# nicholasburden/pymarl

Hardware: NVIDIA B200
Metric: qmix_learner_episodes_per_sec (higher is better)
Workload: dtype bf16 (fp32 accumulate)

## Files before the change

pymarl_b200/csrc/tc_common.cuh:

```cuda
#pragma once
#include <cuda_bf16.h>
#include <stdint.h>

namespace pmb {
namespace tc {

__device__ __forceinline__ uint32_t smem_u32(const void* p) { return (uint32_t)__cvta_generic_to_shared(p); }

__device__ __forceinline__ void mbar_init(uint64_t* bar, uint32_t count) {
    asm volatile("mbarrier.init.shared::cta.b64 [%0], %1;" ::"r"(smem_u32(bar)), "r"(count) : "memory");
}
__device__ __forceinline__ void fence_barrier_init() {
    asm volatile("fence.mbarrier_init.release.cluster;" ::: "memory");
}
__device__ __forceinline__ void mbar_arrive(uint64_t* bar) {
    asm volatile("mbarrier.arrive.shared::cta.b64 _, [%0];" ::"r"(smem_u32(bar)) : "memory");
}
__device__ __forceinline__ void mbar_arrive_expect_tx(uint64_t* bar, uint32_t bytes) {
    asm volatile("mbarrier.arrive.expect_tx.shared::cta.b64 _, [%0], %1;" ::"r"(smem_u32(bar)), "r"(bytes) : "memory");
}
__device__ __forceinline__ bool mbar_try_wait(uint64_t* bar, uint32_t parity) {
    uint32_t ok;
    asm volatile(
        "{\n\t.reg .pred p;\n\t"
// ... 61 lines not shown
__device__ __forceinline__ void tmem_dealloc(uint32_t taddr, uint32_t ncols) {
    asm volatile("tcgen05.dealloc.cta_group::1.sync.aligned.b32 %0, %1;" ::"r"(taddr), "r"(ncols) : "memory");
}
__device__ __forceinline__ void pdl_launch_dependents() { asm volatile("griddepcontrol.launch_dependents;" ::: "memory"); }
__device__ __forceinline__ void pdl_wait() { asm volatile("griddepcontrol.wait;" ::: "memory"); }

__device__ __forceinline__ void tc_fence_before() { asm volatile("tcgen05.fence::before_thread_sync;" ::: "memory"); }
__device__ __forceinline__ void tc_fence_after() { asm volatile("tcgen05.fence::after_thread_sync;" ::: "memory"); }
__device__ __forceinline__ void tmem_wait_ld() { asm volatile("tcgen05.wait::ld.sync.aligned;" ::: "memory"); }

__device__ __forceinline__ void tmem_ld_32x32(uint32_t taddr, uint32_t (&v)[32]) {
    asm volatile(
        "tcgen05.ld.sync.aligned.32x32b.x32.b32 "
        "{%0, %1, %2, %3, %4, %5, %6, %7, %8, %9, %10, %11, %12, %13, %14, %15, "
        "%16, %17, %18, %19, %20, %21, %22, %23, %24, %25, %26, %27, %28, %29, %30, %31}, [%32];"
        : "=r"(v[0]), "=r"(v[1]), "=r"(v[2]), "=r"(v[3]), "=r"(v[4]), "=r"(v[5]), "=r"(v[6]), "=r"(v[7]), "=r"(v[8]),
          "=r"(v[9]), "=r"(v[10]), "=r"(v[11]), "=r"(v[12]), "=r"(v[13]), "=r"(v[14]), "=r"(v[15]), "=r"(v[16]),
          "=r"(v[17]), "=r"(v[18]), "=r"(v[19]), "=r"(v[20]), "=r"(v[21]), "=r"(v[22]), "=r"(v[23]), "=r"(v[24]),
          "=r"(v[25]), "=r"(v[26]), "=r"(v[27]), "=r"(v[28]), "=r"(v[29]), "=r"(v[30]), "=r"(v[31])
        : "r"(taddr)
        : "memory");
}

__device__ __forceinline__ uint64_t umma_desc_sw128(uint32_t smem_addr, uint32_t lbo_bytes, uint32_t sbo_bytes) {
    return (uint64_t)((smem_addr >> 4) & 0x3FFF) | ((uint64_t)((lbo_bytes >> 4) & 0x3FFF) << 16) |
           ((uint64_t)((sbo_bytes >> 4) & 0x3FFF) << 32) | (1ull << 46) | (2ull << 61);
}
__host__ __device__ constexpr uint32_t umma_idesc_bf16(int M, int N, int a_mn_major, int b_mn_major) {
    return (1u << 4) | (1u << 7) | (1u << 10) | ((uint32_t)a_mn_major << 15) | ((uint32_t)b_mn_major << 16) |
           ((uint32_t)(N >> 3) << 17) | ((uint32_t)(M >> 4) << 24);
}

__device__ __forceinline__ void umma_bf16(uint32_t tmem_d, uint64_t a_desc, uint64_t b_desc, uint32_t idesc,
                                          uint32_t accumulate) {
    asm volatile(
        "{\n\t.reg .pred p;\n\t"
        "setp.ne.b32 p, %4, 0;\n\t"
        "tcgen05.mma.cta_group::1.kind::f16 [%0], %1, %2, %3, p;\n\t}"
        :
        : "r"(tmem_d), "l"(a_desc), "l"(b_desc), "r"(idesc), "r"(accumulate)
        : "memory");
}
__device__ __forceinline__ void umma_commit(uint64_t* bar) {
    asm volatile("tcgen05.commit.cta_group::1.mbarrier::arrive::one.shared::cluster.b64 [%0];" ::"r"(smem_u32(bar))
                 : "memory");
}

__device__ __forceinline__ uint32_t pack_bf16x2(float lo, float hi) {
    uint32_t r;
    asm("cvt.rn.bf16x2.f32 %0, %1, %2;" : "=r"(r) : "f"(hi), "f"(lo));
    return r;
}

__host__ __device__ __forceinline__ uint32_t sw128_offset(uint32_t r, uint32_t j) {
    return r * 128u + ((j ^ (r & 7u)) << 4);
}

}
}
```

pymarl_b200/csrc/tc_gemm.cu:

```cuda
#include <cstdlib>
#include <algorithm>
#include "common.cuh"
#include "tc_common.cuh"
#include "mixer_tc.cuh"

namespace pmb {
namespace tc {

constexpr int BM = 128;
constexpr int BK = 64;
constexpr int BN_MAX = 256;
constexpr int STAGES = 4;
constexpr int A_STAGE_BYTES = BM * 128;
constexpr int W_STAGE_BYTES = BN_MAX * 128;
constexpr int N_EPI_WARPS = 4, MMA_WARP = 4, WLOAD_WARP = 5, FIRST_PROD_WARP = 6, N_PROD_WARPS = 8;
constexpr int THREADS = 32 * (FIRST_PROD_WARP + N_PROD_WARPS);
constexpr int SMEM_BYTES = 1024  + STAGES * (A_STAGE_BYTES + W_STAGE_BYTES) + 256;

struct GemmParams {
    const float* A;
    RowMap amap;
    int64_t M;
    int K;
    int n_chunks;
// ... 438 lines not shown
constexpr int RPW = GROUP_ROWS / N_CONV;
constexpr int threads_for(int ns) { return 32 * (PROD_W + ns + N_CONV); }
static_assert(RPW >= 1 && RPW * N_CONV == GROUP_ROWS, "group rows must divide over the converter warps");
}

struct Fc1StreamParams {
    const int64_t* ep_index;
    const float* obs; int64_t obs_sb;
    const __nv_bfloat16* Wp;
    uint8_t* obs_img;
    int64_t R;
    int T, N, O, n_tiles, n_chunks, slot_bytes;
    int fold_id;
    const uint4* tab_act16;
    const float* tab_id;
    const int64_t* actions; int64_t actions_sb;
    const int64_t* filled;  int64_t filled_sb;
    uint8_t* x_on; uint8_t* x_tg;
    uint32_t* relu_mask;
    int use_act;
    int l2_prefetch;
    int n_nets;
    int t0;
};

__device__ __forceinline__ float lds_f32(uint32_t addr) {
    float v;
    asm volatile("ld.shared.f32 %0, [%1];" : "=f"(v) : "r"(addr));
    return v;
}
__device__ __forceinline__ void sts_b32(uint32_t addr, uint32_t v) {
    asm volatile("st.shared.b32 [%0], %1;" ::"r"(addr), "r"(v) : "memory");
}

#ifdef PMB_FC1_PROFILE
__device__ unsigned long long g_fc1_prof[16];
#define TWAIT(idx, bar, par) do { long long _t0 = clock64(); mbar_wait(bar, par); if (lane == 0) prof_acc[idx] += clock64() - _t0; } while (0)
#define TMARK(var) const long long var = clock64()
#define TADD(idx, expr) do { if (lane == 0) prof_acc[idx] += (expr); } while (0)
#else
#define TWAIT(idx, bar, par) mbar_wait(bar, par)
#define TMARK(var)
#define TADD(idx, expr)
#endif
template <int NC, int NS>
__global__ void __launch_bounds__(fs::threads_for(NS), 1) fc1_stream_kernel(Fc1StreamParams P) {
#ifdef PMB_FC1_PROFILE
    long long prof_acc[12] = {0, 0, 0, 0, 0, 0, 0, 0, 0, 0, 0, 0};
    const long long prof_t0 = clock64();
#endif
    using namespace fs;
    extern __shared__ uint8_t smem_raw[];
    uint8_t* smem = reinterpret_cast<uint8_t*>((reinterpret_cast<uintptr_t>(smem_raw) + 1023) & ~(uintptr_t)1023);
    constexpr int N_SLOTS = NS, N_PROD = NS, FIRST_CONV_W = PROD_W + NS;
    constexpr int tile_bytes = NC * A_STAGE_BYTES;
    const int w_chunk = P.n_nets == 2 ? A_STAGE_BYTES : A_STAGE_BYTES / 2;
    uint8_t* w_s = smem;
    uint8_t* a_s = smem + NC * w_chunk;
    uint8_t* stage = a_s + tile_bytes;
    int* rowoff = reinterpret_cast<int*>(stage + N_SLOTS * P.slot_bytes);
    int* rown = rowoff + N_SLOTS * GROUP_ROWS;
    uint64_t* bars = reinterpret_cast<uint64_t*>(rown + N_SLOTS * GROUP_ROWS);
    uint64_t* w_full = bars;
    uint64_t* st_full = bars + 1;
    uint64_t* st_empty = st_full + N_SLOTS;
    uint64_t* a_full = st_empty + N_SLOTS;
    uint64_t* a_free = a_full + 1;
    uint64_t* tfull = a_free + 1;
    uint64_t* tempty = tfull + 2;
    uint32_t* tmem_slot = reinterpret_cast<uint32_t*>(tempty + 2);

    const int warp = threadIdx.x >> 5, lane = threadIdx.x & 31;
    if (threadIdx.x == 0) {
        mbar_init(w_full, 1);
        for (int i = 0; i < N_SLOTS; ++i) { mbar_init(&st_full[i], 1); mbar_init(&st_empty[i], N_CONV); }
        mbar_init(a_full, N_CONV); mbar_init(a_free, 1);
        for (int i = 0; i < 2; ++i) { mbar_init(&tfull[i], 1); mbar_init(&tempty[i], N_EPI); }
        fence_barrier_init();
    }
    if (warp == MMA_W) tmem_alloc(tmem_slot, 256);
    tc_fence_before();
    __syncthreads();
    tc_fence_after();
    const uint32_t tmem_base = *tmem_slot;
    const int64_t n_items = (int64_t)P.T * P.n_tiles;
    pdl_launch_dependents();

    if (warp >= PROD_W && warp < PROD_W + N_PROD) {
        const int pw = warp - PROD_W;
        if (pw == 0 && lane == 0) {
            mbar_arrive_expect_tx(w_full, (uint32_t)(NC * w_chunk));
            for (int c = 0; c < NC; ++c)
                bulk_copy_g2s(w_s + c * w_chunk, reinterpret_cast<const uint8_t*>(P.Wp) + c * A_STAGE_BYTES, (uint32_t)w_chunk, w_full);
        }
        uint32_t git = 0;
        for (int64_t item = blockIdx.x; item < n_items; item += gridDim.x) {
            const int64_t t = item / P.n_tiles, tile = item - t * P.n_tiles;
            for (int g = 0; g < GROUPS; ++g, ++git) {
                const int slot = git % N_SLOTS;
                if (slot != pw) continue;
                TMARK(pp0);
                uint8_t* sl = stage + slot * P.slot_bytes;
                int* ro = rowoff + slot * GROUP_ROWS;
                int* rn = rown + slot * GROUP_ROWS;
                const int64_t p0 = tile * BM + g * GROUP_ROWS;
                int rows_here = P.R - p0 < GROUP_ROWS ? (int)(P.R - p0) : GROUP_ROWS;
                if (rows_here < 0) rows_here = 0;
                const uint32_t b0 = (uint32_t)p0 / (uint32_t)P.N;
                const int n00 = (int)((uint32_t)p0 - b0 * (uint32_t)P.N);
                int first_cnt = P.N - n00;
                if (first_cnt > rows_here) first_cnt = rows_here;
                const int lr = lane == 0 ? 0 : first_cnt + (lane - 1) * P.N;
                int cnt = lane == 0 ? first_cnt : (rows_here - lr < P.N ? rows_here - lr : P.N);
                if (cnt < 0) cnt = 0;
                const int n0 = lane == 0 ? n00 : 0;
                const char* ga = nullptr;
                uint32_t cur = 0, phase = 0, cp_bytes = 0;
                if (cnt > 0) {
                    ga = reinterpret_cast<const char*>(P.obs + ep_row(P.ep_index, (int64_t)b0 + lane) * P.obs_sb +
                                                       ((t + P.t0) * P.N + n0) * (int64_t)P.O);
                    phase = (uint32_t)(reinterpret_cast<uintptr_t>(ga) & 15);
                    cur = (((uint32_t)lr * P.O * 4u + 127u) & ~127u) + 320u * lane + (uint32_t)(reinterpret_cast<uintptr_t>(ga) & 127);
                    cp_bytes = (phase + (uint32_t)cnt * P.O * 4u + 15u) & ~15u;
                }
                const uint32_t tx = __reduce_add_sync(0xffffffffu, cp_bytes);
                if (P.l2_prefetch && cnt > 0 && item + (int64_t)P.l2_prefetch * gridDim.x < n_items) {
                    const int64_t item2 = item + (int64_t)P.l2_prefetch * gridDim.x;
                    const int64_t t2 = item2 / P.n_tiles, tile2 = item2 - t2 * P.n_tiles;
                    const int64_t q0 = tile2 * BM + g * GROUP_ROWS;
                    int rows2 = P.R - q0 < GROUP_ROWS ? (int)(P.R - q0) : GROUP_ROWS;
                    if (rows2 < 0) rows2 = 0;
                    const uint32_t c0 = (uint32_t)q0 / (uint32_t)P.N;
                    const int m00 = (int)((uint32_t)q0 - c0 * (uint32_t)P.N);
                    int fc = P.N - m00;
                    if (fc > rows2) fc = rows2;
                    const int lr2 = lane == 0 ? 0 : fc + (lane - 1) * P.N;
                    int cnt2 = lane == 0 ? fc : (rows2 - lr2 < P.N ? rows2 - lr2 : P.N);
                    if (cnt2 > 0) {
                        const char* gb = reinterpret_cast<const char*>(P.obs + ep_row(P.ep_index, (int64_t)c0 + lane) * P.obs_sb +
                                                                       ((t2 + P.t0) * P.N + (lane == 0 ? m00 : 0)) * (int64_t)P.O);
                        const uintptr_t a0 = (reinterpret_cast<uintptr_t>(gb) + 15) & ~(uintptr_t)15;
                        const uintptr_t a1 = (reinterpret_cast<uintptr_t>(gb) + (uint64_t)cnt2 * P.O * 4) & ~(uintptr_t)15;
                        if (a1 > a0)
                            asm volatile("cp.async.bulk.prefetch.L2.global [%0], %1;" ::"l"(a0), "r"((uint32_t)(a1 - a0)) : "memory");
                    }
                }
                const int rj = lane < first_cnt ? 0 : 1 + (lane - first_cnt) / P.N;
                const int lrj = rj == 0 ? 0 : first_cnt + (rj - 1) * P.N;
                const uint32_t cur_j = __shfl_sync(0xffffffffu, cur, rj & 31);
                TADD(10, clock64() - pp0);
                TWAIT(0, &st_empty[slot], ((git / N_SLOTS) & 1) ^ 1);
                TMARK(pp1);
                if (lane < GROUP_ROWS) {
                    ro[lane] = lane < rows_here ? (int)(cur_j + (uint32_t)(lane - lrj) * P.O * 4u) : -1;
                    rn[lane] = (rj == 0 ? n00 : 0) + (lane - lrj);
                }
                if (cnt > 0) bulk_copy_g2s(sl + cur - phase, ga - phase, cp_bytes, &st_full[slot]);
                __syncwarp();
                if (lane == 0) {
                    if (tx) mbar_arrive_expect_tx(&st_full[slot], tx); else mbar_arrive(&st_full[slot]);
                }
                TADD(11, clock64() - pp1);
            }
        }
    } else if (warp >= FIRST_CONV_W) {
        const int cw = warp - FIRST_CONV_W;
        constexpr int c_last = NC - 1;
        const bool okl0 = c_last * BK + 2 * lane < P.O, okl1 = c_last * BK + 2 * lane + 1 < P.O;
        const int j_pad = c_last * BK + 2 * lane - P.O;
        const uint32_t a_s_u32 = smem_u32(a_s);
        const uint32_t a_base = a_s_u32 + ((uint32_t)(lane >> 2) << 4) + (lane & 3) * 4;
        uint32_t git = 0, ti = 0;
        for (int64_t item = blockIdx.x; item < n_items; item += gridDim.x, ++ti) {
            for (int g = 0; g < GROUPS; ++g, ++git) {
                const int slot = git % N_SLOTS;
                TWAIT(1, &st_full[slot], (git / N_SLOTS) & 1);
                TMARK(pt1);
                const uint32_t sl = smem_u32(stage + slot * P.slot_bytes) + 8u * lane;
                int offs[RPW], nns[RPW];
#pragma unroll
                for (int rr = 0; rr < RPW; ++rr) {
                    offs[rr] = rowoff[slot * GROUP_ROWS + RPW * cw + rr];
                    nns[rr] = rown[slot * GROUP_ROWS + RPW * cw + rr];
                }
                float v0[RPW][NC], v1[RPW][NC];
                {
#pragma unroll
                    for (int rr = 0; rr < RPW; ++rr) {
                        const int off = offs[rr];
                        const bool real = off >= 0;
                        const uint32_t src = sl + (uint32_t)(real ? off : 0);
#pragma unroll
                        for (int c = 0; c < NC; ++c) {
                            v0[rr][c] = 0.f; v1[rr][c] = 0.f;
                            if (real && (c < c_last || okl0)) v0[rr][c] = lds_f32(src + c * 256);
                            if (real && (c < c_last || okl1)) v1[rr][c] = lds_f32(src + c * 256 + 4);
                        }
                    }
                    uint32_t pk[RPW][NC];
#pragma unroll
                    for (int rr = 0; rr < RPW; ++rr) {
                        const int off = offs[rr];
                        const int nn = nns[rr];
                        const bool fold = P.fold_id && off >= 0;
                        const bool hit0 = fold && j_pad >= 0 && (j_pad == nn || j_pad == P.N);
                        const bool hit1 = fold && j_pad + 1 >= 0 && (j_pad + 1 == nn || j_pad + 1 == P.N);
#pragma unroll
                        for (int c = 0; c < NC; ++c) {
                            float a = v0[rr][c], b = v1[rr][c];
                            if (c == c_last) { a = hit0 ? 1.0f : a; b = hit1 ? 1.0f : b; }
                            pk[rr][c] = pack_bf16x2(a, b);
                        }
                    }
                    __syncwarp();
                    if (lane == 0) mbar_arrive(&st_empty[slot]);
                    TMARK(pt2);
                    TADD(6, pt2 - pt1);
                    if (g == 0) TWAIT(2, a_free, (ti & 1) ^ 1);
#pragma unroll
                    for (int rr = 0; rr < RPW; ++rr) {
                        const uint32_t rt = (uint32_t)(g * GROUP_ROWS + RPW * cw + rr);
                        const uint32_t dst = (a_base + rt * 128u) ^ ((rt & 7u) << 4);
#pragma unroll
                        for (int c = 0; c < NC; ++c) sts_b32(dst + c * A_STAGE_BYTES, pk[rr][c]);
                        if (P.obs_img) {
                            uint8_t* img = P.obs_img + item * tile_bytes + (dst - a_s_u32);
#pragma unroll
                            for (int c = 0; c < NC; ++c) __stcs(reinterpret_cast<uint32_t*>(img + c * A_STAGE_BYTES), pk[rr][c]);
                        }
                    }
                    TADD(7, clock64() - pt2);
                }
            }
            fence_proxy_async_smem();
            __syncwarp();
            if (lane == 0) mbar_arrive(a_full);
        }
    } else if (warp == MMA_W) {
        if (lane == 0) {
            const uint32_t idesc = umma_idesc_bf16(BM, 64 * P.n_nets, 0, 0);
            mbar_wait(w_full, 0);
            uint32_t ti = 0;
            for (int64_t item = blockIdx.x; item < n_items; item += gridDim.x, ++ti) {
                const int b = ti & 1;
                TWAIT(3, a_full, ti & 1);
                TWAIT(4, &tempty[b], ((ti >> 1) & 1) ^ 1);
                tc_fence_after();
                const uint32_t tm = tmem_base + 128u * b;
#pragma unroll
                for (int c = 0; c < NC; ++c) {
                    const uint32_t a_addr = smem_u32(a_s + c * A_STAGE_BYTES), w_addr = smem_u32(w_s + c * w_chunk);
#pragma unroll
                    for (int kk = 0; kk < BK / 16; ++kk)
                        umma_bf16(tm, umma_desc_sw128(a_addr + kk * 32, 16, 1024), umma_desc_sw128(w_addr + kk * 32, 16, 1024),
                                  idesc, (c | kk) != 0);
                }
                umma_commit(a_free);
                umma_commit(&tfull[b]);
            }
        }
// ... 51 lines not shown
                        if (tid) {
                            const float4 b0 = __ldg(tid + 2 * q), b1 = __ldg(tid + 2 * q + 1);
                            o[0] += b0.x; o[1] += b0.y; o[2] += b0.z; o[3] += b0.w;
                            o[4] += b1.x; o[5] += b1.y; o[6] += b1.z; o[7] += b1.w;
                        }
#pragma unroll
                        for (int k = 0; k < 8; ++k) {
                            o[k] = fmaxf(o[k], 0.f);
                            mbits |= (o[k] > 0.f ? 1u : 0u) << (8 * q + k);
                        }
                        *reinterpret_cast<uint4*>(tile_img + sw128_offset(r, (uint32_t)(h0 / 8 + q))) =
                            make_uint4(pack_bf16x2(o[0], o[1]), pack_bf16x2(o[2], o[3]), pack_bf16x2(o[4], o[5]),
                                       pack_bf16x2(o[6], o[7]));
                    }
                    if (P.relu_mask && net == 0) P.relu_mask[(item * 2 + (h0 >> 5)) * 128 + r] = mbits;
                }
            }
            tc_fence_before();
            __syncwarp();
            if (lane == 0) mbar_arrive(&tempty[b]);
            a_prev = a_next; n_cur = n_nxt;
        }
    }
#ifdef PMB_FC1_PROFILE
    if (lane == 0) {
        for (int i = 0; i < 8; ++i) if (prof_acc[i]) atomicAdd(&g_fc1_prof[i], (unsigned long long)prof_acc[i]);
        for (int i = 10; i < 12; ++i) if (prof_acc[i]) atomicAdd(&g_fc1_prof[i], (unsigned long long)prof_acc[i]);
        if (threadIdx.x == 0) { atomicAdd(&g_fc1_prof[8], (unsigned long long)(clock64() - prof_t0)); atomicAdd(&g_fc1_prof[9], 1ull); }
    }
#endif
    tc_fence_before();
    __syncthreads();
    if (warp == MMA_W) {
        tc_fence_after();
        tmem_dealloc(tmem_base, 256);
    }
}

}

int64_t tc_packed_elems(int Ncols, int K) {
    int n_chunks = (K + tc::BK - 1) / tc::BK;
    return (int64_t)Ncols * n_chunks * tc::BK;
}

int tc_pack_w(const float* const* ptrs, const int* rows, const int* lds, int nseg, int K, __nv_bfloat16* out,
              cudaStream_t s, int n_chunks_min) {
    tc::PackSegs segs;
    int Ncols = 0;
    segs.nseg = nseg;
    for (int i = 0; i < 4; ++i) {
        segs.ptr[i] = i < nseg ? ptrs[i] : nullptr;
        segs.rows[i] = i < nseg ? rows[i] : 0;
        segs.ld[i] = i < nseg ? lds[i] : 0;
        Ncols += segs.rows[i];
    }
    Ncols = (int)align_up(Ncols, 32);
    int n_chunks = (K + tc::BK - 1) / tc::BK;
// ... 126 lines not shown
                         reinterpret_cast<uint8_t*>(x_on), reinterpret_cast<uint8_t*>(x_tg), t0, nt, d->N, d->A,
                         d->obs_last_action, n_tiles, R, relu_mask};
        const int n_chunks = (d->O + tc::BK - 1) / tc::BK;
        const int slot_bytes = slot_bytes_s;
        const int64_t smem_need = 1024 + 2 * (int64_t)n_chunks * tc::A_STAGE_BYTES + tc::fs::N_SLOTS * (int64_t)slot_bytes +
                                  2 * tc::fs::N_SLOTS * tc::fs::GROUP_ROWS * 4 + 256;
        if (n_chunks <= tc::fs::MAX_CHUNKS && smem_need <= 232448) {
            const int fold_id = n_chunks * tc::BK - d->O >= d->N + 1;
            __nv_bfloat16* tab_act16 = reinterpret_cast<__nv_bfloat16*>(static_cast<char*>(scratch) + wp_bytes + ta_bytes + ti_bytes);
            const int64_t n_pack = (int64_t)128 * n_chunks * 8 + (int64_t)d->A * 128;
            if (!weights_packed) {
                fc1_stream_pack_kernel<<<(unsigned)ceil_div(n_pack, 256), 256, 0, s>>>(
                    on.fc1_w, on.fc1_b, tg.fc1_w, tg.fc1_b, d->O, d->A, d->N, D_in, d->obs_last_action, d->obs_agent_id, fold_id,
                    n_chunks, wp, tab_act16);
                PMB_LAUNCH_CHECK("fc1_stream_pack_kernel");
            }
            tc::Fc1StreamParams Q;
            Q.ep_index = b->ep_index; Q.obs = b->obs; Q.obs_sb = b->obs_sb; Q.Wp = wp; Q.obs_img = obs_img_out; Q.R = R;
            Q.T = nt; Q.N = d->N; Q.O = d->O; Q.n_tiles = n_tiles; Q.n_chunks = n_chunks; Q.slot_bytes = slot_bytes;
            Q.fold_id = fold_id; Q.tab_act16 = reinterpret_cast<const uint4*>(tab_act16); Q.tab_id = tab_id;
            Q.actions = b->actions; Q.actions_sb = b->actions_sb; Q.filled = b->filled; Q.filled_sb = b->filled_sb;
            Q.x_on = reinterpret_cast<uint8_t*>(x_on); Q.x_tg = reinterpret_cast<uint8_t*>(x_tg);
            Q.relu_mask = relu_mask; Q.use_act = d->obs_last_action;
            Q.n_nets = x_tg ? 2 : 1; Q.t0 = t0;
            Q.l2_prefetch = 0;
            { const char* e = getenv("PMB_FC1_PREFETCH"); if (e) Q.l2_prefetch = atoi(e); }
            const int64_t n_items = (int64_t)nt * n_tiles;
            const int grid = (int)(n_items < sm_count() ? n_items : sm_count());
            const int64_t smem_1net = 1024 + (int64_t)n_chunks * (tc::A_STAGE_BYTES / 2) + (int64_t)n_chunks * tc::A_STAGE_BYTES +
                                      tc::fs::N_SLOTS_1NET * (int64_t)slot_bytes + 2 * tc::fs::N_SLOTS_1NET * tc::fs::GROUP_ROWS * 4 + 256;
            const bool wide_ring = Q.n_nets == 1 && smem_1net <= 232448;
#define PMB_FC1_STREAM_LAUNCH(NC)                                                                                            \
    case NC:                                                                                                                 \
        if (wide_ring) {                                                                                                     \
            PMB_SMEM_ATTR((tc::fc1_stream_kernel<NC, tc::fs::N_SLOTS_1NET>), (int)smem_1net);                               \
            PMB_CUDA(launch_pdl(tc::fc1_stream_kernel<NC, tc::fs::N_SLOTS_1NET>, dim3(grid),                                 \
                                dim3(tc::fs::threads_for(tc::fs::N_SLOTS_1NET)), (size_t)smem_1net, s, rollout_pdl_enabled(), Q)); \
        } else {                                                                                                             \
            PMB_SMEM_ATTR((tc::fc1_stream_kernel<NC, tc::fs::N_SLOTS>), (int)smem_need);                                     \
            tc::fc1_stream_kernel<NC, tc::fs::N_SLOTS><<<grid, tc::fs::threads_for(tc::fs::N_SLOTS), (size_t)smem_need, s>>>(Q); \
        }                                                                                                                    \
        break;
            switch (n_chunks) {
                PMB_FC1_STREAM_LAUNCH(1)
                PMB_FC1_STREAM_LAUNCH(2)
                PMB_FC1_STREAM_LAUNCH(3)
                PMB_FC1_STREAM_LAUNCH(4)
                PMB_FC1_STREAM_LAUNCH(5)
            }
#undef PMB_FC1_STREAM_LAUNCH
            PMB_LAUNCH_CHECK("fc1_stream_kernel");
            return PMB_OK;
        }
        if (b->ep_index) { set_error("tc_fc1: ep_index needs the streaming kernel (obs dim <= 320)"); return PMB_ERR_INVALID; }
        return tc::launch_tc_gemm(P, epi, s);
    }
    if (b->ep_index) { set_error("tc_fc1: ep_index is not supported without tile images"); return PMB_ERR_INVALID; }
// ... 94 lines not shown
```

Baseline: 146,300.

## Add TMEM-operand fc1 stream kernel for dual-network learner path

Adds a new fc1 streaming kernel variant that keeps fc1 weights resident in tensor memory and issues tcgen05.mma with a TMEM A operand. It runs online and target networks in one pass, with the epilogue adding last-action table rows and writing ReLU masks and bf16 activations via bulk stores. It also refactors the producer and convert loops into shared device functions. The goal is less shared-memory traffic and a more overlapped pipeline for the two-network case, at the cost of extra TMEM and shared-memory pressure and a more complex code path.

Result: faster. 151,600 (median of 6 runs) (+3.6%).

```diff
diff --git a/pymarl_b200/csrc/tc_common.cuh b/pymarl_b200/csrc/tc_common.cuh
--- a/pymarl_b200/csrc/tc_common.cuh
+++ b/pymarl_b200/csrc/tc_common.cuh
@@ -107,6 +107,20 @@
         : "memory");
 }
 
+__device__ __forceinline__ void tmem_st_32x32(uint32_t taddr, const uint32_t (&v)[32]) {
+    asm volatile(
+        "tcgen05.st.sync.aligned.32x32b.x32.b32 [%0], "
+        "{%1, %2, %3, %4, %5, %6, %7, %8, %9, %10, %11, %12, %13, %14, %15, %16, "
+        "%17, %18, %19, %20, %21, %22, %23, %24, %25, %26, %27, %28, %29, %30, %31, %32};"
+        :
+        : "r"(taddr), "r"(v[0]), "r"(v[1]), "r"(v[2]), "r"(v[3]), "r"(v[4]), "r"(v[5]), "r"(v[6]), "r"(v[7]), "r"(v[8]),
+          "r"(v[9]), "r"(v[10]), "r"(v[11]), "r"(v[12]), "r"(v[13]), "r"(v[14]), "r"(v[15]), "r"(v[16]), "r"(v[17]),
+          "r"(v[18]), "r"(v[19]), "r"(v[20]), "r"(v[21]), "r"(v[22]), "r"(v[23]), "r"(v[24]), "r"(v[25]), "r"(v[26]),
+          "r"(v[27]), "r"(v[28]), "r"(v[29]), "r"(v[30]), "r"(v[31])
+        : "memory");
+}
+__device__ __forceinline__ void tmem_wait_st() { asm volatile("tcgen05.wait::st.sync.aligned;" ::: "memory"); }
+
 __device__ __forceinline__ uint64_t umma_desc_sw128(uint32_t smem_addr, uint32_t lbo_bytes, uint32_t sbo_bytes) {
     return (uint64_t)((smem_addr >> 4) & 0x3FFF) | ((uint64_t)((lbo_bytes >> 4) & 0x3FFF) << 16) |
            ((uint64_t)((sbo_bytes >> 4) & 0x3FFF) << 32) | (1ull << 46) | (2ull << 61);
@@ -126,6 +140,16 @@
         : "r"(tmem_d), "l"(a_desc), "l"(b_desc), "r"(idesc), "r"(accumulate)
         : "memory");
 }
+__device__ __forceinline__ void umma_bf16_ts(uint32_t tmem_d, uint32_t tmem_a, uint64_t b_desc, uint32_t idesc,
+                                             uint32_t accumulate) {
+    asm volatile(
+        "{\n\t.reg .pred p;\n\t"
+        "setp.ne.b32 p, %4, 0;\n\t"
+        "tcgen05.mma.cta_group::1.kind::f16 [%0], [%1], %2, %3, p;\n\t}"
+        :
+        : "r"(tmem_d), "r"(tmem_a), "l"(b_desc), "r"(idesc), "r"(accumulate)
+        : "memory");
+}
 __device__ __forceinline__ void umma_commit(uint64_t* bar) {
     asm volatile("tcgen05.commit.cta_group::1.mbarrier::arrive::one.shared::cluster.b64 [%0];" ::"r"(smem_u32(bar))
                  : "memory");
diff --git a/pymarl_b200/csrc/tc_gemm.cu b/pymarl_b200/csrc/tc_gemm.cu
--- a/pymarl_b200/csrc/tc_gemm.cu
+++ b/pymarl_b200/csrc/tc_gemm.cu
@@ -484,6 +484,7 @@
     int l2_prefetch;
     int n_nets;
     int t0;
+    int n_act;
 };
 
 __device__ __forceinline__ float lds_f32(uint32_t addr) {
@@ -500,17 +501,204 @@
 #define TWAIT(idx, bar, par) do { long long _t0 = clock64(); mbar_wait(bar, par); if (lane == 0) prof_acc[idx] += clock64() - _t0; } while (0)
 #define TMARK(var) const long long var = clock64()
 #define TADD(idx, expr) do { if (lane == 0) prof_acc[idx] += (expr); } while (0)
+#define FC1_PROF_BEGIN long long prof_acc[16] = {}; const long long prof_t0 = clock64()
+#define FC1_PROF_END(ns)                                                                                                  \
+    do {                                                                                                                  \
+        if (lane == 0)                                                                                                    \
+            for (int i = 0; i < 15; ++i)                                                                                  \
+                if (i != 8 && i != 9 && prof_acc[i]) atomicAdd(&g_fc1_prof[i], (unsigned long long)prof_acc[i]);          \
+        if (threadIdx.x == 0) {                                                                                           \
+            atomicAdd(&g_fc1_prof[8], (unsigned long long)(clock64() - prof_t0)); atomicAdd(&g_fc1_prof[9], 1ull);        \
+            atomicAdd(&g_fc1_prof[15], (unsigned long long)(ns));                                                         \
+        }                                                                                                                 \
+    } while (0)
 #else
 #define TWAIT(idx, bar, par) mbar_wait(bar, par)
 #define TMARK(var)
 #define TADD(idx, expr)
+#define FC1_PROF_BEGIN long long prof_acc[16]
+#define FC1_PROF_END(ns) do { } while (0)
 #endif
+struct Fc1Ring {
+    uint8_t* stage;
+    int* rowoff;
+    int* rown;
+    uint64_t* st_full;
+    uint64_t* st_empty;
+};
+
+template <int NC, int NS>
+__device__ __forceinline__ void fc1_produce(const Fc1StreamParams& P, const Fc1Ring& ring, int pw, int lane,
+                                            long long (&prof_acc)[16]) {
+    using namespace fs;
+    constexpr int N_SLOTS = NS;
+    uint8_t* stage = ring.stage;
+    int* rowoff = ring.rowoff;
+    int* rown = ring.rown;
+    uint64_t* st_full = ring.st_full;
+    uint64_t* st_empty = ring.st_empty;
+    const int64_t n_items = (int64_t)P.T * P.n_tiles;
+
+    uint32_t git = 0;
+    for (int64_t item = blockIdx.x; item < n_items; item += gridDim.x) {
+        const int64_t t = item / P.n_tiles, tile = item - t * P.n_tiles;
+        for (int g = 0; g < GROUPS; ++g, ++git) {
+            const int slot = git % N_SLOTS;
+            if (slot != pw) continue;
+            TMARK(pp0);
+            uint8_t* sl = stage + slot * P.slot_bytes;
+            int* ro = rowoff + slot * GROUP_ROWS;
+            int* rn = rown + slot * GROUP_ROWS;
+            const int64_t p0 = tile * BM + g * GROUP_ROWS;
+            int rows_here = P.R - p0 < GROUP_ROWS ? (int)(P.R - p0) : GROUP_ROWS;
+            if (rows_here < 0) rows_here = 0;
+            const uint32_t b0 = (uint32_t)p0 / (uint32_t)P.N;
+            const int n00 = (int)((uint32_t)p0 - b0 * (uint32_t)P.N);
+            int first_cnt = P.N - n00;
+            if (first_cnt > rows_here) first_cnt = rows_here;
+            const int lr = lane == 0 ? 0 : first_cnt + (lane - 1) * P.N;
+            int cnt = lane == 0 ? first_cnt : (rows_here - lr < P.N ? rows_here - lr : P.N);
+            if (cnt < 0) cnt = 0;
+            const int n0 = lane == 0 ? n00 : 0;
+            const char* ga = nullptr;
+            uint32_t cur = 0, phase = 0, cp_bytes = 0;
+            if (cnt > 0) {
+                ga = reinterpret_cast<const char*>(P.obs + ep_row(P.ep_index, (int64_t)b0 + lane) * P.obs_sb +
+                                                   ((t + P.t0) * P.N + n0) * (int64_t)P.O);
+                phase = (uint32_t)(reinterpret_cast<uintptr_t>(ga) & 15);
+                cur = (((uint32_t)lr * P.O * 4u + 127u) & ~127u) + 320u * lane + (uint32_t)(reinterpret_cast<uintptr_t>(ga) & 127);
+                cp_bytes = (phase + (uint32_t)cnt * P.O * 4u + 15u) & ~15u;
+            }
+            const uint32_t tx = __reduce_add_sync(0xffffffffu, cp_bytes);
+            if (P.l2_prefetch && cnt > 0 && item + (int64_t)P.l2_prefetch * gridDim.x < n_items) {
+                const int64_t item2 = item + (int64_t)P.l2_prefetch * gridDim.x;
+                const int64_t t2 = item2 / P.n_tiles, tile2 = item2 - t2 * P.n_tiles;
+                const int64_t q0 = tile2 * BM + g * GROUP_ROWS;
+                int rows2 = P.R - q0 < GROUP_ROWS ? (int)(P.R - q0) : GROUP_ROWS;
+                if (rows2 < 0) rows2 = 0;
+                const uint32_t c0 = (uint32_t)q0 / (uint32_t)P.N;
+                const int m00 = (int)((uint32_t)q0 - c0 * (uint32_t)P.N);
+                int fc = P.N - m00;
+                if (fc > rows2) fc = rows2;
+                const int lr2 = lane == 0 ? 0 : fc + (lane - 1) * P.N;
+                int cnt2 = lane == 0 ? fc : (rows2 - lr2 < P.N ? rows2 - lr2 : P.N);
+                if (cnt2 > 0) {
+                    const char* gb = reinterpret_cast<const char*>(P.obs + ep_row(P.ep_index, (int64_t)c0 + lane) * P.obs_sb +
+                                                                   ((t2 + P.t0) * P.N + (lane == 0 ? m00 : 0)) * (int64_t)P.O);
+                    const uintptr_t a0 = (reinterpret_cast<uintptr_t>(gb) + 15) & ~(uintptr_t)15;
+                    const uintptr_t a1 = (reinterpret_cast<uintptr_t>(gb) + (uint64_t)cnt2 * P.O * 4) & ~(uintptr_t)15;
+                    if (a1 > a0)
+                        asm volatile("cp.async.bulk.prefetch.L2.global [%0], %1;" ::"l"(a0), "r"((uint32_t)(a1 - a0)) : "memory");
+                }
+            }
+            const int rj = lane < first_cnt ? 0 : 1 + (lane - first_cnt) / P.N;
+            const int lrj = rj == 0 ? 0 : first_cnt + (rj - 1) * P.N;
+            const uint32_t cur_j = __shfl_sync(0xffffffffu, cur, rj & 31);
+            TADD(10, clock64() - pp0);
+            TWAIT(0, &st_empty[slot], ((git / N_SLOTS) & 1) ^ 1);
+            TMARK(pp1);
+            if (lane < GROUP_ROWS) {
+                ro[lane] = lane < rows_here ? (int)(cur_j + (uint32_t)(lane - lrj) * P.O * 4u) : -1;
+                rn[lane] = (rj == 0 ? n00 : 0) + (lane - lrj);
+            }
+            if (cnt > 0) bulk_copy_g2s(sl + cur - phase, ga - phase, cp_bytes, &st_full[slot]);
+            __syncwarp();
+            if (lane == 0) {
+                if (tx) mbar_arrive_expect_tx(&st_full[slot], tx); else mbar_arrive(&st_full[slot]);
+            }
+            TADD(11, clock64() - pp1);
+        }
+    }
+}
+
+template <int NC, int NS>
+__device__ __forceinline__ void fc1_convert(const Fc1StreamParams& P, const Fc1Ring& ring, uint8_t* a_s, uint64_t* a_free,
+                                            uint64_t* a_full, int cw, int lane, long long (&prof_acc)[16]) {
+    using namespace fs;
+    constexpr int N_SLOTS = NS;
+    constexpr int tile_bytes = NC * A_STAGE_BYTES;
+    uint8_t* stage = ring.stage;
+    int* rowoff = ring.rowoff;
+    int* rown = ring.rown;
+    uint64_t* st_full = ring.st_full;
+    uint64_t* st_empty = ring.st_empty;
+    const int64_t n_items = (int64_t)P.T * P.n_tiles;
+    constexpr int c_last = NC - 1;
+    const bool okl0 = c_last * BK + 2 * lane < P.O, okl1 = c_last * BK + 2 * lane + 1 < P.O;
+    const int j_pad = c_last * BK + 2 * lane - P.O;
+    const uint32_t a_s_u32 = smem_u32(a_s);
+    const uint32_t a_base = a_s_u32 + ((uint32_t)(lane >> 2) << 4) + (lane & 3) * 4;
+    uint32_t git = 0, ti = 0;
+    for (int64_t item = blockIdx.x; item < n_items; item += gridDim.x, ++ti) {
+        for (int g = 0; g < GROUPS; ++g, ++git) {
+            const int slot = git % N_SLOTS;
+            TWAIT(1, &st_full[slot], (git / N_SLOTS) & 1);
+            TMARK(pt1);
+            const uint32_t sl = smem_u32(stage + slot * P.slot_bytes) + 8u * lane;
+            int offs[RPW], nns[RPW];
+#pragma unroll
+            for (int rr = 0; rr < RPW; ++rr) {
+                offs[rr] = rowoff[slot * GROUP_ROWS + RPW * cw + rr];
+                nns[rr] = rown[slot * GROUP_ROWS + RPW * cw + rr];
+            }
+            float v0[RPW][NC], v1[RPW][NC];
+            {
+#pragma unroll
+                for (int rr = 0; rr < RPW; ++rr) {
+                    const int off = offs[rr];
+                    const bool real = off >= 0;
+                    const uint32_t src = sl + (uint32_t)(real ? off : 0);
+#pragma unroll
+                    for (int c = 0; c < NC; ++c) {
+                        v0[rr][c] = 0.f; v1[rr][c] = 0.f;
+                        if (real && (c < c_last || okl0)) v0[rr][c] = lds_f32(src + c * 256);
+                        if (real && (c < c_last || okl1)) v1[rr][c] = lds_f32(src + c * 256 + 4);
+                    }
+                }
+                uint32_t pk[RPW][NC];
+#pragma unroll
+                for (int rr = 0; rr < RPW; ++rr) {
+                    const int off = offs[rr];
+                    const int nn = nns[rr];
+                    const bool fold = P.fold_id && off >= 0;
+                    const bool hit0 = fold && j_pad >= 0 && (j_pad == nn || j_pad == P.N);
+                    const bool hit1 = fold && j_pad + 1 >= 0 && (j_pad + 1 == nn || j_pad + 1 == P.N);
+#pragma unroll
+                    for (int c = 0; c < NC; ++c) {
+                        float a = v0[rr][c], b = v1[rr][c];
+                        if (c == c_last) { a = hit0 ? 1.0f : a; b = hit1 ? 1.0f : b; }
+                        pk[rr][c] = pack_bf16x2(a, b);
+                    }
+                }
+                __syncwarp();
+                if (lane == 0) mbar_arrive(&st_empty[slot]);
+                TMARK(pt2);
+                TADD(6, pt2 - pt1);
+                if (g == 0) TWAIT(2, a_free, (ti & 1) ^ 1);
+#pragma unroll
+                for (int rr = 0; rr < RPW; ++rr) {
+                    const uint32_t rt = (uint32_t)(g * GROUP_ROWS + RPW * cw + rr);
+                    const uint32_t dst = (a_base + rt * 128u) ^ ((rt & 7u) << 4);
+#pragma unroll
+                    for (int c = 0; c < NC; ++c) sts_b32(dst + c * A_STAGE_BYTES, pk[rr][c]);
+                    if (P.obs_img) {
+                        uint8_t* img = P.obs_img + item * tile_bytes + (dst - a_s_u32);
+#pragma unroll
+                        for (int c = 0; c < NC; ++c) __stcs(reinterpret_cast<uint32_t*>(img + c * A_STAGE_BYTES), pk[rr][c]);
+                    }
+                }
+                TADD(7, clock64() - pt2);
+            }
+        }
+        fence_proxy_async_smem();
+        __syncwarp();
+        if (lane == 0) mbar_arrive(a_full);
+    }
+}
+
 template <int NC, int NS>
 __global__ void __launch_bounds__(fs::threads_for(NS), 1) fc1_stream_kernel(Fc1StreamParams P) {
-#ifdef PMB_FC1_PROFILE
-    long long prof_acc[12] = {0, 0, 0, 0, 0, 0, 0, 0, 0, 0, 0, 0};
-    const long long prof_t0 = clock64();
-#endif
+    FC1_PROF_BEGIN;
     using namespace fs;
     extern __shared__ uint8_t smem_raw[];
     uint8_t* smem = reinterpret_cast<uint8_t*>((reinterpret_cast<uintptr_t>(smem_raw) + 1023) & ~(uintptr_t)1023);
@@ -546,6 +734,7 @@
     tc_fence_after();
     const uint32_t tmem_base = *tmem_slot;
     const int64_t n_items = (int64_t)P.T * P.n_tiles;
+    const Fc1Ring ring{stage, rowoff, rown, st_full, st_empty};
     pdl_launch_dependents();
 
     if (warp >= PROD_W && warp < PROD_W + N_PROD) {
@@ -555,149 +744,9 @@
             for (int c = 0; c < NC; ++c)
                 bulk_copy_g2s(w_s + c * w_chunk, reinterpret_cast<const uint8_t*>(P.Wp) + c * A_STAGE_BYTES, (uint32_t)w_chunk, w_full);
         }
-        uint32_t git = 0;
-        for (int64_t item = blockIdx.x; item < n_items; item += gridDim.x) {
-            const int64_t t = item / P.n_tiles, tile = item - t * P.n_tiles;
-            for (int g = 0; g < GROUPS; ++g, ++git) {
-                const int slot = git % N_SLOTS;
-                if (slot != pw) continue;
-                TMARK(pp0);
-                uint8_t* sl = stage + slot * P.slot_bytes;
-                int* ro = rowoff + slot * GROUP_ROWS;
-                int* rn = rown + slot * GROUP_ROWS;
-                const int64_t p0 = tile * BM + g * GROUP_ROWS;
-                int rows_here = P.R - p0 < GROUP_ROWS ? (int)(P.R - p0) : GROUP_ROWS;
-                if (rows_here < 0) rows_here = 0;
-                const uint32_t b0 = (uint32_t)p0 / (uint32_t)P.N;
-                const int n00 = (int)((uint32_t)p0 - b0 * (uint32_t)P.N);
-                int first_cnt = P.N - n00;
-                if (first_cnt > rows_here) first_cnt = rows_here;
-                const int lr = lane == 0 ? 0 : first_cnt + (lane - 1) * P.N;
-                int cnt = lane == 0 ? first_cnt : (rows_here - lr < P.N ? rows_here - lr : P.N);
-                if (cnt < 0) cnt = 0;
-                const int n0 = lane == 0 ? n00 : 0;
-                const char* ga = nullptr;
-                uint32_t cur = 0, phase = 0, cp_bytes = 0;
-                if (cnt > 0) {
-                    ga = reinterpret_cast<const char*>(P.obs + ep_row(P.ep_index, (int64_t)b0 + lane) * P.obs_sb +
-                                                       ((t + P.t0) * P.N + n0) * (int64_t)P.O);
-                    phase = (uint32_t)(reinterpret_cast<uintptr_t>(ga) & 15);
-                    cur = (((uint32_t)lr * P.O * 4u + 127u) & ~127u) + 320u * lane + (uint32_t)(reinterpret_cast<uintptr_t>(ga) & 127);
-                    cp_bytes = (phase + (uint32_t)cnt * P.O * 4u + 15u) & ~15u;
-                }
-                const uint32_t tx = __reduce_add_sync(0xffffffffu, cp_bytes);
-                if (P.l2_prefetch && cnt > 0 && item + (int64_t)P.l2_prefetch * gridDim.x < n_items) {
-                    const int64_t item2 = item + (int64_t)P.l2_prefetch * gridDim.x;
-                    const int64_t t2 = item2 / P.n_tiles, tile2 = item2 - t2 * P.n_tiles;
-                    const int64_t q0 = tile2 * BM + g * GROUP_ROWS;
-                    int rows2 = P.R - q0 < GROUP_ROWS ? (int)(P.R - q0) : GROUP_ROWS;
-                    if (rows2 < 0) rows2 = 0;
-                    const uint32_t c0 = (uint32_t)q0 / (uint32_t)P.N;
-                    const int m00 = (int)((uint32_t)q0 - c0 * (uint32_t)P.N);
-                    int fc = P.N - m00;
-                    if (fc > rows2) fc = rows2;
-                    const int lr2 = lane == 0 ? 0 : fc + (lane - 1) * P.N;
-                    int cnt2 = lane == 0 ? fc : (rows2 - lr2 < P.N ? rows2 - lr2 : P.N);
-                    if (cnt2 > 0) {
-                        const char* gb = reinterpret_cast<const char*>(P.obs + ep_row(P.ep_index, (int64_t)c0 + lane) * P.obs_sb +
-                                                                       ((t2 + P.t0) * P.N + (lane == 0 ? m00 : 0)) * (int64_t)P.O);
-                        const uintptr_t a0 = (reinterpret_cast<uintptr_t>(gb) + 15) & ~(uintptr_t)15;
-                        const uintptr_t a1 = (reinterpret_cast<uintptr_t>(gb) + (uint64_t)cnt2 * P.O * 4) & ~(uintptr_t)15;
-                        if (a1 > a0)
-                            asm volatile("cp.async.bulk.prefetch.L2.global [%0], %1;" ::"l"(a0), "r"((uint32_t)(a1 - a0)) : "memory");
-                    }
-                }
-                const int rj = lane < first_cnt ? 0 : 1 + (lane - first_cnt) / P.N;
-                const int lrj = rj == 0 ? 0 : first_cnt + (rj - 1) * P.N;
-                const uint32_t cur_j = __shfl_sync(0xffffffffu, cur, rj & 31);
-                TADD(10, clock64() - pp0);
-                TWAIT(0, &st_empty[slot], ((git / N_SLOTS) & 1) ^ 1);
-                TMARK(pp1);
-                if (lane < GROUP_ROWS) {
-                    ro[lane] = lane < rows_here ? (int)(cur_j + (uint32_t)(lane - lrj) * P.O * 4u) : -1;
-                    rn[lane] = (rj == 0 ? n00 : 0) + (lane - lrj);
-                }
-                if (cnt > 0) bulk_copy_g2s(sl + cur - phase, ga - phase, cp_bytes, &st_full[slot]);
-                __syncwarp();
-                if (lane == 0) {
-                    if (tx) mbar_arrive_expect_tx(&st_full[slot], tx); else mbar_arrive(&st_full[slot]);
-                }
-                TADD(11, clock64() - pp1);
-            }
-        }
+        fc1_produce<NC, NS>(P, ring, pw, lane, prof_acc);
     } else if (warp >= FIRST_CONV_W) {
-        const int cw = warp - FIRST_CONV_W;
-        constexpr int c_last = NC - 1;
-        const bool okl0 = c_last * BK + 2 * lane < P.O, okl1 = c_last * BK + 2 * lane + 1 < P.O;
-        const int j_pad = c_last * BK + 2 * lane - P.O;
-        const uint32_t a_s_u32 = smem_u32(a_s);
-        const uint32_t a_base = a_s_u32 + ((uint32_t)(lane >> 2) << 4) + (lane & 3) * 4;
-        uint32_t git = 0, ti = 0;
-        for (int64_t item = blockIdx.x; item < n_items; item += gridDim.x, ++ti) {
-            for (int g = 0; g < GROUPS; ++g, ++git) {
-                const int slot = git % N_SLOTS;
-                TWAIT(1, &st_full[slot], (git / N_SLOTS) & 1);
-                TMARK(pt1);
-                const uint32_t sl = smem_u32(stage + slot * P.slot_bytes) + 8u * lane;
-                int offs[RPW], nns[RPW];
-#pragma unroll
-                for (int rr = 0; rr < RPW; ++rr) {
-                    offs[rr] = rowoff[slot * GROUP_ROWS + RPW * cw + rr];
-                    nns[rr] = rown[slot * GROUP_ROWS + RPW * cw + rr];
-                }
-                float v0[RPW][NC], v1[RPW][NC];
-                {
-#pragma unroll
-                    for (int rr = 0; rr < RPW; ++rr) {
-                        const int off = offs[rr];
-                        const bool real = off >= 0;
-                        const uint32_t src = sl + (uint32_t)(real ? off : 0);
-#pragma unroll
-                        for (int c = 0; c < NC; ++c) {
-                            v0[rr][c] = 0.f; v1[rr][c] = 0.f;
-                            if (real && (c < c_last || okl0)) v0[rr][c] = lds_f32(src + c * 256);
-                            if (real && (c < c_last || okl1)) v1[rr][c] = lds_f32(src + c * 256 + 4);
-                        }
-                    }
-                    uint32_t pk[RPW][NC];
-#pragma unroll
-                    for (int rr = 0; rr < RPW; ++rr) {
-                        const int off = offs[rr];
-                        const int nn = nns[rr];
-                        const bool fold = P.fold_id && off >= 0;
-                        const bool hit0 = fold && j_pad >= 0 && (j_pad == nn || j_pad == P.N);
-                        const bool hit1 = fold && j_pad + 1 >= 0 && (j_pad + 1 == nn || j_pad + 1 == P.N);
-#pragma unroll
-                        for (int c = 0; c < NC; ++c) {
-                            float a = v0[rr][c], b = v1[rr][c];
-                            if (c == c_last) { a = hit0 ? 1.0f : a; b = hit1 ? 1.0f : b; }
-                            pk[rr][c] = pack_bf16x2(a, b);
-                        }
-                    }
-                    __syncwarp();
-                    if (lane == 0) mbar_arrive(&st_empty[slot]);
-                    TMARK(pt2);
-                    TADD(6, pt2 - pt1);
-                    if (g == 0) TWAIT(2, a_free, (ti & 1) ^ 1);
-#pragma unroll
-                    for (int rr = 0; rr < RPW; ++rr) {
-                        const uint32_t rt = (uint32_t)(g * GROUP_ROWS + RPW * cw + rr);
-                        const uint32_t dst = (a_base + rt * 128u) ^ ((rt & 7u) << 4);
-#pragma unroll
-                        for (int c = 0; c < NC; ++c) sts_b32(dst + c * A_STAGE_BYTES, pk[rr][c]);
-                        if (P.obs_img) {
-                            uint8_t* img = P.obs_img + item * tile_bytes + (dst - a_s_u32);
-#pragma unroll
-                            for (int c = 0; c < NC; ++c) __stcs(reinterpret_cast<uint32_t*>(img + c * A_STAGE_BYTES), pk[rr][c]);
-                        }
-                    }
-                    TADD(7, clock64() - pt2);
-                }
-            }
-            fence_proxy_async_smem();
-            __syncwarp();
-            if (lane == 0) mbar_arrive(a_full);
-        }
+        fc1_convert<NC, NS>(P, ring, a_s, a_free, a_full, warp - FIRST_CONV_W, lane, prof_acc);
     } else if (warp == MMA_W) {
         if (lane == 0) {
             const uint32_t idesc = umma_idesc_bf16(BM, 64 * P.n_nets, 0, 0);
@@ -795,18 +844,216 @@
             a_prev = a_next; n_cur = n_nxt;
         }
     }
-#ifdef PMB_FC1_PROFILE
-    if (lane == 0) {
-        for (int i = 0; i < 8; ++i) if (prof_acc[i]) atomicAdd(&g_fc1_prof[i], (unsigned long long)prof_acc[i]);
-        for (int i = 10; i < 12; ++i) if (prof_acc[i]) atomicAdd(&g_fc1_prof[i], (unsigned long long)prof_acc[i]);
-        if (threadIdx.x == 0) { atomicAdd(&g_fc1_prof[8], (unsigned long long)(clock64() - prof_t0)); atomicAdd(&g_fc1_prof[9], 1ull); }
-    }
-#endif
+    FC1_PROF_END(NS);
     tc_fence_before();
     __syncthreads();
     if (warp == MMA_W) {
         tc_fence_after();
         tmem_dealloc(tmem_base, 256);
+    }
+}
+
+
+namespace fs {
+constexpr int N_SLOTS_TS = 5;
+constexpr int TS_TMEM_W = 256;
+}
+
+__device__ __forceinline__ void epi_bar_sync() { asm volatile("bar.sync 1, 128;" ::: "memory"); }
+
+template <int NC>
+__global__ void __launch_bounds__(fs::threads_for(fs::N_SLOTS_TS), 1) fc1_stream_ts_kernel(Fc1StreamParams P) {
+    FC1_PROF_BEGIN;
+    using namespace fs;
+    constexpr int NS = N_SLOTS_TS, FIRST_CONV_W = PROD_W + NS;
+    extern __shared__ uint8_t smem_raw[];
+    uint8_t* smem = reinterpret_cast<uint8_t*>((reinterpret_cast<uintptr_t>(smem_raw) + 1023) & ~(uintptr_t)1023);
+    uint8_t* a_s = smem;
+    uint8_t* xs = a_s + NC * A_STAGE_BYTES;
+    uint8_t* stage = xs + 2 * A_STAGE_BYTES;
+    float* tab_s = reinterpret_cast<float*>(stage + NS * P.slot_bytes);
+    int* prev_s = reinterpret_cast<int*>(tab_s + P.n_act * 128);
+    int* rowoff = prev_s + 2 * BM;
+    int* rown = rowoff + NS * GROUP_ROWS;
+    uint64_t* bars = reinterpret_cast<uint64_t*>(rown + NS * GROUP_ROWS);
+    uint64_t* w_full = bars;
+    uint64_t* st_full = bars + 1;
+    uint64_t* st_empty = st_full + NS;
+    uint64_t* a_full = st_empty + NS;
+    uint64_t* a_free = a_full + 1;
+    uint64_t* tfull = a_free + 1;
+    uint64_t* tempty = tfull + 2;
+    uint32_t* tmem_slot = reinterpret_cast<uint32_t*>(tempty + 2);
+
+    const int warp = threadIdx.x >> 5, lane = threadIdx.x & 31;
+    if (threadIdx.x == 0) {
+        mbar_init(w_full, N_EPI);
+        for (int i = 0; i < NS; ++i) { mbar_init(&st_full[i], 1); mbar_init(&st_empty[i], N_CONV); }
+        mbar_init(a_full, N_CONV); mbar_init(a_free, 1);
+        for (int i = 0; i < 2; ++i) { mbar_init(&tfull[i], 1); mbar_init(&tempty[i], N_EPI); }
+        fence_barrier_init();
+    }
+    if (warp == MMA_W) tmem_alloc(tmem_slot, 512);
+    tc_fence_before();
+    __syncthreads();
+    tc_fence_after();
+    const Fc1Ring ring{stage, rowoff, rown, st_full, st_empty};
+
+    if (warp >= PROD_W && warp < PROD_W + NS) {
+        fc1_produce<NC, NS>(P, ring, warp - PROD_W, lane, prof_acc);
+    } else if (warp >= FIRST_CONV_W) {
+        fc1_convert<NC, NS>(P, ring, a_s, a_free, a_full, warp - FIRST_CONV_W, lane, prof_acc);
+    } else if (warp == MMA_W) {
+        if (lane == 0) {
+            const uint32_t tmem_base = *tmem_slot;
+            const int64_t n_items = (int64_t)P.T * P.n_tiles;
+            const uint32_t idesc = umma_idesc_bf16(BM, BM, 0, 0);
+            mbar_wait(w_full, 0);
+            tc_fence_after();
+            uint32_t ti = 0;
+            for (int64_t item = blockIdx.x; item < n_items; item += gridDim.x, ++ti) {
+                const int b = ti & 1;
+                TWAIT(3, a_full, ti & 1);
+                TWAIT(4, &tempty[b], ((ti >> 1) & 1) ^ 1);
+                tc_fence_after();
+                const uint32_t tm = tmem_base + 128u * b;
+#pragma unroll
+                for (int c = 0; c < NC; ++c) {
+                    const uint32_t a_addr = smem_u32(a_s + c * A_STAGE_BYTES);
+#pragma unroll
+                    for (int kk = 0; kk < BK / 16; ++kk)
+                        umma_bf16_ts(tm, tmem_base + TS_TMEM_W + (uint32_t)(c * (BK / 16) + kk) * 8u,
+                                     umma_desc_sw128(a_addr + kk * 32, 16, 1024), idesc, (c | kk) != 0);
+                }
+                umma_commit(a_free);
+                umma_commit(&tfull[b]);
+            }
+        }
+    } else {
+        const int hl = warp * 32 + lane;
+        const int net = warp >> 1;
+        const uint32_t tmem_base = *tmem_slot;
+        const int64_t n_items = (int64_t)P.T * P.n_tiles;
+        TMARK(pe0);
+        {
+            const uint8_t* wrow = reinterpret_cast<const uint8_t*>(P.Wp) + hl * 128;
+#pragma unroll
+            for (int c = 0; c < NC; ++c) {
+                uint32_t v[32];
+#pragma unroll
+                for (int j = 0; j < 8; ++j) {
+                    const uint4 u = __ldg(reinterpret_cast<const uint4*>(wrow + c * A_STAGE_BYTES + ((j ^ (hl & 7)) << 4)));
+                    v[4 * j] = u.x; v[4 * j + 1] = u.y; v[4 * j + 2] = u.z; v[4 * j + 3] = u.w;
+                }
+                tmem_st_32x32(tmem_base + TS_TMEM_W + 32u * c + ((uint32_t)(warp * 32) << 16), v);
+            }
+            tmem_wait_st();
+            tc_fence_before();
+            __syncwarp();
+            if (lane == 0) mbar_arrive(w_full);
+        }
+        {
+            const uint16_t* ta = reinterpret_cast<const uint16_t*>(P.tab_act16);
+            for (int i = hl; i < P.n_act * 128; i += 128) tab_s[i] = __uint_as_float((uint32_t)__ldg(ta + i) << 16);
+        }
+        TADD(14, clock64() - pe0);
+        auto fetch_prev = [&](int64_t item) {
+            if (item >= n_items) return -2;
+            const int64_t t = item / P.n_tiles, tile = item - t * P.n_tiles;
+            const int64_t p = tile * BM + hl;
+            if (p >= P.R) return -2;
+            const int64_t b = p / P.N;
+            const int n = (int)(p - b * P.N);
+            const int64_t tb = t + P.t0;
+            if (!P.use_act || tb == 0) return -1;
+            const int64_t be = ep_row(P.ep_index, b);
+            const int64_t f = __ldg(P.filled + be * P.filled_sb + (tb - 1));
+            const int a = (int)__ldg(P.actions + be * P.actions_sb + (tb - 1) * P.N + n);
+            return f != 0 ? a : -1;
+        };
+        int a_prev = fetch_prev(blockIdx.x);
+        const uint32_t xs_u32 = smem_u32(xs + net * A_STAGE_BYTES);
+        const uint32_t h2 = (uint32_t)(hl & 62);
+        const uint32_t xs_lane = xs_u32 + (h2 & 7) * 2;
+        const uint32_t tab_u32 = smem_u32(tab_s + hl);
+        uint32_t ti = 0;
+        for (int64_t item = blockIdx.x; item < n_items; item += gridDim.x, ++ti) {
+            const int b = ti & 1;
+            const int a_next = fetch_prev(item + gridDim.x);
+            const uint32_t pv_u32 = smem_u32(prev_s + b * BM);
+            prev_s[b * BM + hl] = a_prev;
+            TMARK(pe1);
+            if (threadIdx.x == 0) bulk_wait_group_read<0>();
+            epi_bar_sync();
+            TADD(12, clock64() - pe1);
+            TWAIT(5, &tfull[b], (ti >> 1) & 1);
+            tc_fence_after();
+            TMARK(pe2);
+            const int64_t tile = item % P.n_tiles;
+            const int rows_valid = P.R - tile * BM < BM ? (int)(P.R - tile * BM) : BM;
+            const uint32_t taddr = tmem_base + 128u * b + ((uint32_t)(warp * 32) << 16);
+#pragma unroll 1
+            for (int g = 0; g < 4; ++g) {
+                uint32_t v[32];
+                tmem_ld_32x32(taddr + 32 * g, v);
+                tmem_wait_ld();
+                if (g == 3) {
+                    tc_fence_before();
+                    __syncwarp();
+                    if (lane == 0) mbar_arrive(&tempty[b]);
+                }
+                int pa[32];
+#pragma unroll
+                for (int q = 0; q < 8; ++q) {
+                    int4 p4;
+                    asm volatile("ld.shared.v4.s32 {%0, %1, %2, %3}, [%4];"
+                                 : "=r"(p4.x), "=r"(p4.y), "=r"(p4.z), "=r"(p4.w) : "r"(pv_u32 + (uint32_t)(32 * g + 4 * q) * 4u));
+                    pa[4 * q] = p4.x; pa[4 * q + 1] = p4.y; pa[4 * q + 2] = p4.z; pa[4 * q + 3] = p4.w;
+                }
+                float o[32];
+                uint32_t mword = 0;
+#pragma unroll
+                for (int e = 0; e < 32; ++e) {
+                    const int a = pa[e];
+                    const float t = lds_f32(tab_u32 + (uint32_t)(a > 0 ? a : 0) * 512u);
+                    float x = __uint_as_float(v[e]);
+                    x = a >= 0 ? x + t : x;
+                    x = fmaxf(x, 0.f);
+                    o[e] = x;
+                    const uint32_t bal = __ballot_sync(0xffffffffu, x > 0.f);
+                    mword = lane == e ? bal : mword;
+                }
+                if (net == 0 && P.relu_mask && 32 * g + lane < rows_valid)
+                    P.relu_mask[(item * 2 + warp) * 128 + 32 * g + lane] = mword;
+#pragma unroll
+                for (int e = 0; e < 32; ++e) {
+                    if (e & 4) continue;
+                    const bool odd = lane & 1;
+                    const float send = odd ? o[e] : o[e + 4];
+                    const float recv = __shfl_xor_sync(0xffffffffu, send, 1);
+                    const uint32_t w = odd ? pack_bf16x2(recv, o[e + 4]) : pack_bf16x2(o[e], recv);
+                    const uint32_t row = (uint32_t)(32 * g + e + (odd ? 4 : 0));
+                    sts_b32(xs_lane + sw128_offset(row, h2 >> 3), w);
+                }
+            }
+            fence_proxy_async_smem();
+            epi_bar_sync();
+            if (threadIdx.x == 0) {
+                bulk_copy_s2g(P.x_on + item * A_STAGE_BYTES, xs, (uint32_t)rows_valid * 128u);
+                bulk_copy_s2g(P.x_tg + item * A_STAGE_BYTES, xs + A_STAGE_BYTES, (uint32_t)rows_valid * 128u);
+                bulk_commit_group();
+            }
+            TADD(13, clock64() - pe2);
+            a_prev = a_next;
+        }
+        if (threadIdx.x == 0) bulk_wait_group<0>();
+    }
+    FC1_PROF_END(NS);
+    tc_fence_before();
+    __syncthreads();
+    if (warp == MMA_W) {
+        tc_fence_after();
+        tmem_dealloc(*tmem_slot, 512);
     }
 }
 
@@ -979,7 +1226,7 @@
             Q.actions = b->actions; Q.actions_sb = b->actions_sb; Q.filled = b->filled; Q.filled_sb = b->filled_sb;
             Q.x_on = reinterpret_cast<uint8_t*>(x_on); Q.x_tg = reinterpret_cast<uint8_t*>(x_tg);
             Q.relu_mask = relu_mask; Q.use_act = d->obs_last_action;
-            Q.n_nets = x_tg ? 2 : 1; Q.t0 = t0;
+            Q.n_nets = x_tg ? 2 : 1; Q.t0 = t0; Q.n_act = d->A;
             Q.l2_prefetch = 0;
             { const char* e = getenv("PMB_FC1_PREFETCH"); if (e) Q.l2_prefetch = atoi(e); }
             const int64_t n_items = (int64_t)nt * n_tiles;
@@ -987,9 +1234,16 @@
             const int64_t smem_1net = 1024 + (int64_t)n_chunks * (tc::A_STAGE_BYTES / 2) + (int64_t)n_chunks * tc::A_STAGE_BYTES +
                                       tc::fs::N_SLOTS_1NET * (int64_t)slot_bytes + 2 * tc::fs::N_SLOTS_1NET * tc::fs::GROUP_ROWS * 4 + 256;
             const bool wide_ring = Q.n_nets == 1 && smem_1net <= 232448;
+            const int64_t smem_ts = 1024 + (int64_t)(n_chunks + 2) * tc::A_STAGE_BYTES + tc::fs::N_SLOTS_TS * (int64_t)slot_bytes +
+                                    (int64_t)d->A * 128 * 4 + 2 * tc::BM * 4 + 2 * tc::fs::N_SLOTS_TS * tc::fs::GROUP_ROWS * 4 + 256;
+            const char* e_ts = getenv("PMB_FC1_TS");
+            const bool use_ts = Q.n_nets == 2 && fold_id && smem_ts <= 232448 && !(e_ts && e_ts[0] == '0');
 #define PMB_FC1_STREAM_LAUNCH(NC)                                                                                            \
     case NC:                                                                                                                 \
-        if (wide_ring) {                                                                                                     \
+        if (use_ts) {                                                                                                        \
+            PMB_SMEM_ATTR((tc::fc1_stream_ts_kernel<NC>), (int)smem_ts);                                                     \
+            tc::fc1_stream_ts_kernel<NC><<<grid, tc::fs::threads_for(tc::fs::N_SLOTS_TS), (size_t)smem_ts, s>>>(Q);          \
+        } else if (wide_ring) {                                                                                              \
             PMB_SMEM_ATTR((tc::fc1_stream_kernel<NC, tc::fs::N_SLOTS_1NET>), (int)smem_1net);                               \
             PMB_CUDA(launch_pdl(tc::fc1_stream_kernel<NC, tc::fs::N_SLOTS_1NET>, dim3(grid),                                 \
                                 dim3(tc::fs::threads_for(tc::fs::N_SLOTS_1NET)), (size_t)smem_1net, s, rollout_pdl_enabled(), Q)); \
```
